# landrumb/ParlayANN

Hardware: AMD Instinct MI355X
Metric: QPS @ recall@10>=0.95, SIFT-1M d=128 beam=64; achieved HBM GB/s vs roofline (higher is better)
Workload: dtype f16; 1 GPU; SIFT-1M-shaped batched beam search: 1000000x128 integer-valued fp32->f16 base, 10000 queries/step/GPU, beam=64 k=10 cut=1.35 start=0, prebuilt Vamana R=64 L=128 alpha=1.15 x2 passes (built on device); n=1000000, d=128, nq_per_gpu=10000, beam=64, k=10, parallelism=query-sharded x1, index replicated, no collective

## Files before the change

parlayann_amd/csrc/beam_search.hip:

```cpp
#include <cstdio>
#include <cstdlib>
#include <vector>

#include "pann_device.h"

namespace pann {

#ifndef PANN_GU
#define PANN_GU 4
#endif
#ifndef PANN_GU_B128
#define PANN_GU_B128(LPC, NCH1) 4
#endif
#ifndef PANN_MINWAVES
#define PANN_MINWAVES 1
#endif
#ifndef PANN_B128_PAIR
#define PANN_B128_PAIR 0
#endif
#ifndef PANN_B128_PAIR_CODES
#define PANN_B128_PAIR_CODES 1
#endif
#ifndef PANN_B64_PREFETCH
#define PANN_B64_PREFETCH 1
// ... 375 lines not shown
          degsum += __popcll(am);
          const bool seen = filter_update<HASH_LDS>(H, hmask, act, a, lane, reinterpret_cast<uint8_t*>(Hl));
          const bool keep = act && !seen && ((int64_t)a != self);
          const uint64_t km = __ballot(keep);
          const uint32_t m = __popcll(km);
          if (keep) PANN_PL[lanes_below(km, lane)] = a;
          dcmps += m;
          PANN_WSYNC();
          PANN_STAMP(2);
          if (m) c = gather_distances<DT, METRIC, LPC, NCH1, PANN_GU>(P, qreg, qlds, PANN_PL, m, cutoff_ord, C, c, lane);
          PANN_WSYNC();
          PANN_STAMP(3);
        }
        PANN_WSYNC();
        const bool skip = (c == 0) || (P.skip_enabled && c < beam / 8 && more_unvisited);
        do_merge = !skip;
      }
      if (do_merge) {
        {
          for (uint32_t j0 = 0; j0 < c; j0 += PANN_WAVE) {
            const uint32_t j = j0 + lane;
            uint64_t key = KEY_INF;
            uint32_t p = 0;
            if (j < c) {
              key = C[j];
              bool dead = false;
              for (uint32_t i = 0; i < j; i++) dead |= (C[i] == key);
              p = lower_bound_lds(F, f, key);
              dead |= (p < f && F[p] == key);
              if (dead) key = KEY_INF;
            }
            PANN_WSYNC();
            if (j < c) { C[j] = key; CP[j] = (uint16_t)p; }
            PANN_WSYNC();
          }
          uint32_t nvalid = 0;
          for (uint32_t j0 = 0; j0 < c; j0 += PANN_WAVE) {
            const uint32_t j = j0 + lane;
            const uint64_t key = j < c ? C[j] : KEY_INF;
            nvalid += __popcll(__ballot(key != KEY_INF));
            if (key != KEY_INF) {
              uint32_t r = 0;
              for (uint32_t i = 0; i < c; i++) r += (C[i] < key) ? 1u : 0u;
              const uint32_t pos = r + CP[j];
              if (pos < beam) {
                uint32_t flag = 0u;
                for (uint32_t t = 0; t < ndrop; t++)
                  flag |= (__hip_atomic_load(DL + t, __ATOMIC_RELAXED, PANN_PRIVATE_SCOPE) == key) ? 2u : 0u;
                NF[pos] = key; NFv[pos] = (uint8_t)flag;
              }
            }
          }
          for (uint32_t e0 = 0; e0 < f; e0 += PANN_WAVE) {
            const uint32_t e = e0 + lane;
            if (e < f) {
              const uint64_t key = F[e];
              uint32_t below = 0;
              for (uint32_t i = 0; i < c; i++) below += (C[i] < key) ? 1u : 0u;
              const uint32_t pos = e + below;
              if (pos < beam) { NF[pos] = key; NFv[pos] = Fv[e]; }
            }
          }
          PANN_WSYNC();
          const uint32_t f_old = f;
          uint32_t f_new = min(f_old + nvalid, beam);
          if (!first && P.cut_enabled && f_new > P.k) {
            const float dk = key_dist(NF[P.k]);
            const float thr = (float)(P.cut * (double)dk);
            const uint64_t thr_key = (uint64_t)f2ord(thr) << 32;
            uint32_t ub = 0;
            for (uint32_t e0 = 0; e0 < f_new; e0 += PANN_WAVE) {
              const uint32_t e = e0 + lane;
              ub += __popcll(__ballot(e < f_new && NF[e] <= thr_key));
            }
            f_new = max(ub, f_old);
          }
          if (f_new == beam) {
            ndrop = 0;
          } else if (P.cut_enabled && !first) {
            for (uint32_t e0 = 0; e0 < f_old; e0 += PANN_WAVE) {
              const uint32_t e = e0 + lane;
              bool lost = false;
              uint64_t key = 0;
              if (e < f_old && Fv[e] == 1) {
                key = F[e];
                uint32_t below = 0;
                for (uint32_t i = 0; i < c; i++) below += (C[i] < key) ? 1u : 0u;
                lost = (e + below) >= f_new;
              }
              const uint64_t lm = __ballot(lost);
              if (lost) {
                const uint32_t at = ndrop + lanes_below(lm, lane);
                if (at < P.dcap) DL[at] = key; else atomicOr(P.status, 2u);
              }
              ndrop = min(ndrop + (uint32_t)__popcll(lm), P.dcap);
            }
            __builtin_amdgcn_s_waitcnt(0);
          }
          { uint64_t* t = F; F = NF; NF = t; uint8_t* tv = Fv; Fv = NFv; NFv = tv; }
          f = f_new;
          c = 0;
          PANN_WSYNC();
        }
      }
      PANN_STAMP(4);
      first = false;
    }

    const size_t qo = (size_t)qi * P.out.out_k;
    for (uint32_t j = lane; j < P.out.out_k; j += PANN_WAVE) {
      const bool ok = j < f;
      uint64_t key = 0ull;
      if (ok) key = F[j];
      if (P.out.ids) P.out.ids[qo + j] = ok ? key_id(key) : SENTINEL;
      if (P.out.dists) P.out.dists[qo + j] = ok ? key_dist(key) : __builtin_inff();
    }
#ifdef PANN_STAMPS
    if (lane == 0 && P.stamps) for (int i = 0; i < 8; i++) P.stamps[(size_t)qi * 8 + i] = stamp_sum[i];
#endif
    if (lane == 0) {
      if (P.out.frontier_size) P.out.frontier_size[qi] = f;
      if (P.out.visited_count) P.out.visited_count[qi] = nvis;
      if (P.out.dist_cmps) P.out.dist_cmps[qi] = dcmps;
      if (P.out.degree_sum) P.out.degree_sum[qi] = degsum;
    }
    PANN_WSYNC();
    if constexpr (HASH_LDS) break;
    else {
      slot = 0;
      if (lane == 0) slot = atomicAdd(P.work_counter, 1u);
      slot = __builtin_amdgcn_readfirstlane(slot);
    }
  }
}

template <int DT, int METRIC, int LPC, bool NCH1>
__global__ void __launch_bounds__(PANN_WAVE, PANN_MINWAVES_B64) beam_search_b64_kernel(BSParams P) {
  const int lane = threadIdx.x;
  extern __shared__ __align__(16) uint8_t smem[];
  uint64_t* S = reinterpret_cast<uint64_t*>(smem);
  uint64_t* C = S + 64;
  uint8_t* Sv = reinterpret_cast<uint8_t*>(C + P.ccap);
  uint4* qlds = reinterpret_cast<uint4*>(Sv + 64);
  uint32_t* H = reinterpret_cast<uint32_t*>(qlds + (NCH1 ? 0 : P.nch * LPC));
  uint32_t* Pl = reinterpret_cast<uint32_t*>(S);

  const uint32_t hsize = 1u << P.bits, hmask = hsize - 1u;
  const uint32_t beam = P.beam;
  const uint32_t BIG_ORD = f2ord(2147483648.0f);
  const uint32_t qi = P.order ? P.order[blockIdx.x] : blockIdx.x;
  if (blockIdx.x >= P.prio_start) __builtin_amdgcn_s_setprio(3);

  for (uint32_t i = lane; i < hsize; i += PANN_WAVE) H[i] = SENTINEL;
  const int64_t self = P.query_ids ? (int64_t)P.query_ids[qi] : -1;
  const uint8_t* qrow = P.query_ids ? P.points + (uint64_t)self * P.pstride : P.queries + (uint64_t)qi * P.qstride;
  QReg<DT> qreg{};
  load_query<DT, LPC, NCH1>(qrow, P.dbytes, P.nch, qreg, qlds, lane);
  PANN_WSYNC();

  uint32_t f = 0, c = 0, nvis = 0, dcmps = P.nstarts, degsum = 0, ndrop = 0;
  uint64_t fkey = KEY_INF;
  uint32_t fflag = 0;
  uint64_t* DL = P.dropped + (size_t)qi * P.dcap;
#ifdef PANN_STAMPS
  unsigned long long stamp_sum[8] = {0, 0, 0, 0, 0, 0, 0, 0}, stamp_prev;
  asm volatile("s_memtime %0\n\ts_waitcnt lgkmcnt(0)" : "=s"(stamp_prev)::"memory");
#endif

  {
    const bool act = lane < (int)P.nstarts;
    const uint32_t a = act ? P.starts[(size_t)qi * P.starts_stride + lane] : 0u;
    (void)filter_update<true>(H, hmask, act, a, lane);
    if (act) Pl[lane] = a;
    PANN_WSYNC();
    c = gather_distances<DT, METRIC, LPC, NCH1, 4>(P, qreg, qlds, Pl, P.nstarts, 0xFFFFFFFFu, C, c, lane);
    PANN_WSYNC();
  }

  uint32_t pref_id = SENTINEL, pref_row = SENTINEL;
  bool first = true;
  for (;;) {
    bool do_merge = first;
    if (!first) {
      const uint64_t um = __ballot(lane < (int)f && fflag == 0);
      if (um == 0ull || nvis >= P.limit) break;
      const int cur_idx = __ffsll((unsigned long long)um) - 1;
      const bool more_unvisited = (um & (um - 1)) != 0ull;
      PANN_STAMP(0);
      const uint64_t cur_key = readlane64(fkey, cur_idx);
      const uint32_t cur = key_id(cur_key);
      if (lane == cur_idx) fflag = 1;
      if (lane == 0 && P.out.visited_cap) {
        if (nvis < P.out.visited_cap) {
          if (P.out.visited_ids) P.out.visited_ids[(size_t)qi * P.out.visited_cap + nvis] = cur;
          if (P.out.visited_dists) P.out.visited_dists[(size_t)qi * P.out.visited_cap + nvis] = key_dist(cur_key);
        } else {
          atomicOr(P.status, 1u);
        }
      }
      nvis++;
      uint32_t cutoff_ord = BIG_ORD;
      if (f == beam) cutoff_ord = (uint32_t)(readlane64(fkey, (int)f - 1) >> 32);

      asm volatile("s_waitcnt vmcnt(0)" : "+v"(pref_row));
      const bool pref_hit = PANN_B64_PREFETCH && (pref_id == cur);
      const uint32_t pref_val = pref_row;
      pref_id = SENTINEL;
      const uint64_t rest1 = um & (um - 1);
      const bool pair_try = PANN_B64_PAIR && P.skip_enabled && rest1 != 0ull && P.gstride <= PANN_WAVE && nvis < P.limit;
      if (PANN_B64_PREFETCH) {
        const uint64_t rest = pair_try ? (rest1 & (rest1 - 1)) : rest1;
        if (rest) {
          pref_id = key_id(readlane64(fkey, __ffsll((unsigned long long)rest) - 1));
          const uint32_t* np = P.graph + (size_t)pref_id * P.gstride + min((uint32_t)lane, P.gstride - 1);
          asm volatile("global_load_dword %0, %1, off" : "=v"(pref_row) : "v"(np));
        }
      }

      const uint32_t* row = P.graph + (size_t)cur * P.gstride;
      if (pair_try) {
        const int idx2 = __ffsll((unsigned long long)rest1) - 1;
        const bool more_after2 = (rest1 & (rest1 - 1)) != 0ull;
        const uint64_t key2 = readlane64(fkey, idx2);
        const uint32_t cur2 = key_id(key2);
        uint32_t a1 = SENTINEL, a2 = SENTINEL;
        if (lane < (int)P.gstride) {
          a1 = pref_hit ? pref_val : row[lane];
          a2 = P.graph[(size_t)cur2 * P.gstride + lane];
        }
        const bool act1 = (a1 != SENTINEL) && ((uint32_t)lane < P.degree_limit);
        const bool act2 = (a2 != SENTINEL) && ((uint32_t)lane < P.degree_limit);
        PANN_STAMP(1);
        const bool seen1 = filter_update<true>(H, hmask, act1, a1, lane);
        FilterUndo u2;
        const bool seen2 = filter_update<true>(H, hmask, act2, a2, lane, nullptr, 0, LdsPart{nullptr, 0, 0}, &u2);
        const bool keep1 = act1 && !seen1 && ((int64_t)a1 != self);
        const bool keep2 = act2 && !seen2 && ((int64_t)a2 != self);
        const uint64_t km1 = __ballot(keep1), km2 = __ballot(keep2);
        const uint32_t m1 = __popcll(km1), m2 = __popcll(km2);
        const bool both = (c + m1 + m2 <= P.ccap);
        if (keep1) Pl[lanes_below(km1, lane)] = a1;
        if (both && keep2) Pl[m1 + lanes_below(km2, lane)] = a2;
        PANN_WSYNC();
        PANN_STAMP(2);
        uint32_t c_after1 = c;
        if (both) {
          if (m1 + m2) c = gather_distances_split<DT, METRIC, LPC, NCH1, PANN_GU, true>(P, qreg, qlds, Pl, m1 + m2, m1, cutoff_ord, C, c, lane, &c_after1);
        } else {
          if (m1) c = gather_distances<DT, METRIC, LPC, NCH1, PANN_GU>(P, qreg, qlds, Pl, m1, cutoff_ord, C, c, lane);
          c_after1 = c;
        }
        PANN_WSYNC();
        PANN_STAMP(3);
        const bool two = both && (c_after1 == 0 || c_after1 < beam / 8);
        if (!two) { c = c_after1; filter_undo<true>(H, u2, 0, LdsPart{nullptr, 0, 0}); }
        if (two) {
          if (lane == idx2) fflag = 1;
          if (lane == 0 && P.out.visited_cap) {
            if (nvis < P.out.visited_cap) {
              if (P.out.visited_ids) P.out.visited_ids[(size_t)qi * P.out.visited_cap + nvis] = cur2;
              if (P.out.visited_dists) P.out.visited_dists[(size_t)qi * P.out.visited_cap + nvis] = key_dist(key2);
            } else {
              atomicOr(P.status, 1u);
            }
          }
          nvis++;
        }
        degsum += __popcll(__ballot(act1)) + (two ? __popcll(__ballot(act2)) : 0u);
        dcmps += m1 + (two ? m2 : 0u);
        const bool more_left = two ? more_after2 : true;
        const bool skip = (c == 0) || (c < beam / 8 && more_left);
        do_merge = !skip;
      } else {
      for (uint32_t i0 = 0; i0 < P.gstride; i0 += PANN_WAVE) {
        const uint32_t i = i0 + lane;
        uint32_t a = SENTINEL;
        if (i0 == 0 && pref_hit) { if (i < P.gstride) a = pref_val; }
        else if (i < P.gstride) a = row[i];
        const bool act = (a != SENTINEL) && (i < P.degree_limit);
        const uint64_t am = __ballot(act);
        PANN_STAMP(1);
        if (am == 0ull) break;
        degsum += __popcll(am);
        const bool seen = filter_update<true>(H, hmask, act, a, lane);
        const bool keep = act && !seen && ((int64_t)a != self);
        const uint64_t km = __ballot(keep);
        const uint32_t m = __popcll(km);
        if (keep) Pl[lanes_below(km, lane)] = a;
        dcmps += m;
        PANN_WSYNC();
        PANN_STAMP(2);
        if (m) c = gather_distances<DT, METRIC, LPC, NCH1, PANN_GU>(P, qreg, qlds, Pl, m, cutoff_ord, C, c, lane);
        PANN_WSYNC();
        PANN_STAMP(3);
      }
      const bool skip = (c == 0) || (P.skip_enabled && c < beam / 8 && more_unvisited);
      do_merge = !skip;
      }
    }
    if (do_merge) {
      const uint32_t f_old = f;
      const bool track = P.cut_enabled && !first;
      uint32_t lt = 0;
      for (uint32_t c0 = 0; c0 < c; c0 += PANN_WAVE) {
        const uint32_t cc = min(c - c0, (uint32_t)PANN_WAVE);
        const uint64_t ckey = (lane < (int)cc) ? C[c0 + lane] : KEY_INF;
        const bool fl = lane < (int)f;
        uint32_t myp = 0, rank_c = 0, below_f = 0;
        uint64_t live_mask = 0;
        const uint64_t vmask = __ballot(fl);
        const uint32_t cid = (uint32_t)ckey, fid = (uint32_t)fkey;
        for (uint32_t i = 0; i < cc; i++) {
          const uint64_t kk = readlane64(ckey, (int)i);
          const uint32_t kid = (uint32_t)kk;
          const bool g = kk < fkey;
          const uint64_t gtm = __ballot(g);
          const uint64_t eqm = __ballot(fid == kid);
          const uint64_t dupm = __ballot(cid == kid) & ((1ull << i) - 1ull);
          if (eqm == 0ull && dupm == 0ull) {
            live_mask |= 1ull << i;
            if (lane == (int)i) myp = f - (uint32_t)__popcll(gtm & vmask);
            rank_c += (kk < ckey) ? 1u : 0u;
            below_f += g ? 1u : 0u;
          }
        }
        const uint32_t nvalid = __popcll(live_mask);
        const bool clive = (lane < (int)cc) && ((live_mask >> lane) & 1ull);
        const uint32_t cpos = rank_c + myp, fpos = (uint32_t)lane + below_f;
        if (clive && cpos < beam) {
          uint32_t flag = 0u;
          for (uint32_t t = 0; t < ndrop; t++)
            flag |= (__hip_atomic_load(DL + t, __ATOMIC_RELAXED, PANN_PRIVATE_SCOPE) == ckey) ? 2u : 0u;
          S[cpos] = ckey; Sv[cpos] = (uint8_t)flag;
        }
        if (fl && fpos < beam) { S[fpos] = fkey; Sv[fpos] = (uint8_t)fflag; }
        if (track) {
          const bool lost = fl && fflag == 1u && fpos >= beam;
          const uint64_t lm = __ballot(lost);
          if (lost) {
            const uint32_t at = ndrop + lt + lanes_below(lm, lane);
            if (at < P.dcap) DL[at] = fkey; else atomicOr(P.status, 2u);
          }
          lt += __popcll(lm);
        }
        PANN_WSYNC();
        f = min(f + nvalid, beam);
        fkey = (lane < (int)f) ? S[lane] : KEY_INF;
        fflag = (lane < (int)f) ? (uint32_t)Sv[lane] : 0u;
        PANN_WSYNC();
      }
      uint32_t f_new = f;
      if (!first && P.cut_enabled && f_new > P.k) {
        const float dk = key_dist(readlane64(fkey, (int)P.k));
        const float thr = (float)(P.cut * (double)dk);
        const uint64_t thr_key = (uint64_t)f2ord(thr) << 32;
        const uint32_t ub = __popcll(__ballot(lane < (int)f_new && fkey <= thr_key));
        f_new = max(ub, f_old);
      }
      if (f_new == beam) {
        ndrop = 0;
      } else if (track) {
        const bool lost = lane >= (int)f_new && lane < (int)f && fflag == 1u;
        const uint64_t lm = __ballot(lost);
        if (lost) {
          const uint32_t at = ndrop + lt + lanes_below(lm, lane);
          if (at < P.dcap) DL[at] = fkey; else atomicOr(P.status, 2u);
        }
        lt += __popcll(lm);
        ndrop = min(ndrop + lt, P.dcap);
        if (lt) __builtin_amdgcn_s_waitcnt(0);
      }
      f = f_new;
      if (lane >= (int)f) { fkey = KEY_INF; fflag = 0u; }
      c = 0;
    }
    PANN_STAMP(4);
    first = false;
  }
  asm volatile("s_waitcnt vmcnt(0)" : "+v"(pref_row));

  const size_t qo = (size_t)qi * P.out.out_k;
  if (lane < (int)P.out.out_k) {
    const bool ok = lane < (int)f;
    if (P.out.ids) P.out.ids[qo + lane] = ok ? key_id(fkey) : SENTINEL;
    if (P.out.dists) P.out.dists[qo + lane] = ok ? key_dist(fkey) : __builtin_inff();
  }
#ifdef PANN_STAMPS
  if (lane == 0 && P.stamps) for (int i = 0; i < 8; i++) P.stamps[(size_t)qi * 8 + i] = stamp_sum[i];
#endif
  if (lane == 0) {
    if (P.out.frontier_size) P.out.frontier_size[qi] = f;
    if (P.out.visited_count) P.out.visited_count[qi] = nvis;
    if (P.out.dist_cmps) P.out.dist_cmps[qi] = dcmps;
    if (P.out.degree_sum) P.out.degree_sum[qi] = degsum;
  }
}

template <int DT, int METRIC, int LPC, bool NCH1, bool HASH_LDS, bool CODES = false>
__global__ void __launch_bounds__(PANN_WAVE) beam_search_b128_kernel(BSParams P) {
  static_assert(!CODES || HASH_LDS, "the code table lives in LDS");
  constexpr int RB = 2;
  const int lane = threadIdx.x;
  extern __shared__ __align__(16) uint8_t smem[];
  uint64_t* S = reinterpret_cast<uint64_t*>(smem);
  uint64_t* C = S + 64 * RB;
  uint8_t* Sv = reinterpret_cast<uint8_t*>(C + P.ccap);
  uint4* qlds = reinterpret_cast<uint4*>(Sv + 64 * RB);
  uint32_t* Hl = reinterpret_cast<uint32_t*>(qlds + (NCH1 ? 0 : P.nch * LPC));
  uint8_t* T = reinterpret_cast<uint8_t*>(S);
  uint32_t* Pl = reinterpret_cast<uint32_t*>(S);

  const uint32_t hsize = 1u << P.bits, hmask = hsize - 1u;
  const uint32_t beam = P.beam;
  const uint32_t BIG_ORD = f2ord(2147483648.0f);
  const LdsPart Lp{reinterpret_cast<uint8_t*>(Hl), HASH_LDS ? 0u : (P.hsplit == 3 ? hsize : P.hsplit ? hsize - (hsize >> P.hsplit) : 0u), P.p24};
  uint32_t slot = blockIdx.x;
  if constexpr (!HASH_LDS) {
    slot = 0;
    if (lane == 0) slot = atomicAdd(P.work_counter, 1u);
    slot = __builtin_amdgcn_readfirstlane(slot);
  }
  while (slot < P.nq) {
  const uint32_t qi = P.order ? P.order[slot] : slot;
  uint32_t* H = HASH_LDS ? Hl : P.hash_global + ((size_t)blockIdx.x << P.bits);
  const uint32_t hb = HASH_LDS ? 0u : P.hsplit;
  uint8_t* const P8 = reinterpret_cast<uint8_t*>(Hl);
  uint32_t* const P4 = Hl + (hsize >> 2);
  if constexpr (CODES) {
    for (uint32_t i = lane; i < (hsize >> 2) + (hsize >> 3); i += PANN_WAVE) Hl[i] = 0xFFFFFFFFu;
  } else {
    if (hb != 3) for (uint32_t i = lane; i < (hsize >> hb); i += PANN_WAVE) hstore<HASH_LDS>(H, i, SENTINEL);
    if (hb) lds_part_clear(Lp, lane);
  }
  const int64_t self = P.query_ids ? (int64_t)P.query_ids[qi] : -1;
  const uint8_t* qrow = P.query_ids ? P.points + (uint64_t)self * P.pstride : P.queries + (uint64_t)qi * P.qstride;
  QReg<DT> qreg{};
  load_query<DT, LPC, NCH1>(qrow, P.dbytes, P.nch, qreg, qlds, lane);
  hsync<HASH_LDS>();

  uint32_t f = 0, c = 0, nvis = 0, dcmps = P.nstarts, degsum = 0, ndrop = 0;
  uint64_t fkey[RB] = {KEY_INF, KEY_INF};
  uint32_t fflag[RB] = {0, 0};
  uint64_t* DL = P.dropped + (size_t)qi * P.dcap;
#ifdef PANN_STAMPS
  unsigned long long stamp_sum[8] = {0, 0, 0, 0, 0, 0, 0, 0}, stamp_prev;
  asm volatile("s_memtime %0\n\ts_waitcnt lgkmcnt(0)" : "=s"(stamp_prev)::"memory");
#endif
  auto entry_key = [&](uint32_t e) -> uint64_t {
    return (e < 64) ? readlane64(fkey[0], (int)e) : readlane64(fkey[1], (int)e - 64);
  };

  {
    const bool act = lane < (int)P.nstarts;
    const uint32_t a = act ? P.starts[(size_t)qi * P.starts_stride + lane] : 0u;
    if constexpr (CODES) (void)filter_update_codes(P8, P4, hmask, act, a, act ? (uint32_t)P.rank16[a] : 0u, lane, T);
    else (void)filter_update<HASH_LDS>(H, hmask, act, a, lane, T, hb, Lp);
    if (act) Pl[lane] = a;
    PANN_WSYNC();
    c = gather_distances<DT, METRIC, LPC, NCH1, 4, false>(P, qreg, qlds, Pl, P.nstarts, 0xFFFFFFFFu, C, c, lane);
    PANN_WSYNC();
  }

  uint32_t pref_id = SENTINEL, pref_row = SENTINEL, pref_code = 0;
  bool first = true;
  for (;;) {
    bool do_merge = first;
    if (!first) {
      const uint64_t um0 = __ballot(lane < (int)f && fflag[0] == 0);
      const uint64_t um1 = __ballot(lane + 64 < (int)f && fflag[1] == 0);
      if ((um0 | um1) == 0ull || nvis >= P.limit) break;
      const int cur_idx = um0 ? __ffsll((unsigned long long)um0) - 1 : 64 + __ffsll((unsigned long long)um1) - 1;
      const bool more_unvisited = (__popcll(um0) + __popcll(um1)) > 1;
      PANN_STAMP(0);
      const uint64_t cur_key = entry_key((uint32_t)cur_idx);
      const uint32_t cur = key_id(cur_key);
      if ((CODES ? PANN_B128_PAIR_CODES : PANN_B128_PAIR) && P.skip_enabled && more_unvisited && P.gstride <= PANN_WAVE && nvis + 1 < P.limit) {
        uint64_t r0 = um0, r1 = um1;
        if (r0) r0 &= r0 - 1; else r1 &= r1 - 1;
        const int idx2 = r0 ? __ffsll((unsigned long long)r0) - 1 : 64 + __ffsll((unsigned long long)r1) - 1;
        if (r0) r0 &= r0 - 1; else r1 &= r1 - 1;
        const bool more_after2 = (r0 | r1) != 0ull;
        const uint64_t key2 = entry_key((uint32_t)idx2);
        const uint32_t cur2 = key_id(key2);
        uint32_t cutoff2 = BIG_ORD;
        if (f == beam) cutoff2 = (uint32_t)(entry_key(f - 1) >> 32);
        uint32_t a1 = SENTINEL, a2 = SENTINEL, code1 = 0, code2 = 0;
        if (lane < (int)P.gstride) {
          a1 = (pref_id == cur) ? pref_row : P.graph[(size_t)cur * P.gstride + lane];
          a2 = P.graph[(size_t)cur2 * P.gstride + lane];
          if constexpr (CODES) {
            code1 = (pref_id == cur) ? pref_code : (uint32_t)P.gcode[(size_t)cur * P.gstride + lane];
            code2 = P.gcode[(size_t)cur2 * P.gstride + lane];
          }
        }
        pref_id = SENTINEL;
        const bool act1 = (a1 != SENTINEL) && ((uint32_t)lane < P.degree_limit);
        const bool act2 = (a2 != SENTINEL) && ((uint32_t)lane < P.degree_limit);
        FilterUndo u2;
        bool seen1, seen2;
        if constexpr (CODES) {
          seen1 = filter_update_codes(P8, P4, hmask, act1, a1, code1, lane, T);
          seen2 = filter_update_codes(P8, P4, hmask, act2, a2, code2, lane, T, &u2);
        } else {
          seen1 = filter_update<HASH_LDS>(H, hmask, act1, a1, lane, T, hb, Lp);
          seen2 = filter_update<HASH_LDS>(H, hmask, act2, a2, lane, T, hb, Lp, &u2);
        }
        const bool keep1 = act1 && !seen1 && ((int64_t)a1 != self);
        const bool keep2 = act2 && !seen2 && ((int64_t)a2 != self);
        const uint64_t km1 = __ballot(keep1), km2 = __ballot(keep2);
        const uint32_t m1 = __popcll(km1), m2 = __popcll(km2);
        const bool both = (c + m1 + m2 <= P.ccap);
        if (keep1) Pl[lanes_below(km1, lane)] = a1;
        if (both && keep2) Pl[m1 + lanes_below(km2, lane)] = a2;
        PANN_WSYNC();
        uint32_t c_after1 = c;
        if (both) {
          if (m1 + m2) c = gather_distances_split<DT, METRIC, LPC, NCH1, PANN_GU_B128(LPC, NCH1)>(P, qreg, qlds, Pl, m1 + m2, m1, cutoff2, C, c, lane, &c_after1);
        } else {
          if (m1) c = gather_distances<DT, METRIC, LPC, NCH1, PANN_GU_B128(LPC, NCH1), false>(P, qreg, qlds, Pl, m1, cutoff2, C, c, lane);
          c_after1 = c;
        }
        PANN_WSYNC();
        const bool two = both && (c_after1 == 0 || c_after1 < beam / 8);
        if (!two) {
          c = c_after1;
          if constexpr (CODES) filter_undo_codes(P8, P4, u2);
          else filter_undo<HASH_LDS>(H, u2, hb, Lp);
        }
        if (cur_idx < 64) { if (lane == cur_idx) fflag[0] = 1; } else { if (lane == cur_idx - 64) fflag[1] = 1; }
        if (two) { if (idx2 < 64) { if (lane == idx2) fflag[0] = 1; } else { if (lane == idx2 - 64) fflag[1] = 1; } }
        if (lane == 0 && P.out.visited_cap) {
          const uint32_t nv = two ? 2u : 1u;
          if (nvis + nv <= P.out.visited_cap) {
            const size_t at = (size_t)qi * P.out.visited_cap + nvis;
            if (P.out.visited_ids) { P.out.visited_ids[at] = cur; if (two) P.out.visited_ids[at + 1] = cur2; }
            if (P.out.visited_dists) { P.out.visited_dists[at] = key_dist(cur_key); if (two) P.out.visited_dists[at + 1] = key_dist(key2); }
          } else {
            atomicOr(P.status, 1u);
          }
        }
        nvis += two ? 2u : 1u;
        degsum += __popcll(__ballot(act1)) + (two ? __popcll(__ballot(act2)) : 0u);
        dcmps += m1 + (two ? m2 : 0u);
        const bool more_left = two ? more_after2 : true;
        const bool skip = (c == 0) || (c < beam / 8 && more_left);
        do_merge = !skip;
      } else {
      if (cur_idx < 64) { if (lane == cur_idx) fflag[0] = 1; } else { if (lane == cur_idx - 64) fflag[1] = 1; }
      if (lane == 0 && P.out.visited_cap) {
        if (nvis < P.out.visited_cap) {
          if (P.out.visited_ids) P.out.visited_ids[(size_t)qi * P.out.visited_cap + nvis] = cur;
          if (P.out.visited_dists) P.out.visited_dists[(size_t)qi * P.out.visited_cap + nvis] = key_dist(cur_key);
        } else {
          atomicOr(P.status, 1u);
        }
      }
      nvis++;
      uint32_t cutoff_ord = BIG_ORD;
      if (f == beam) cutoff_ord = (uint32_t)(entry_key(f - 1) >> 32);

      const uint32_t* row = P.graph + (size_t)cur * P.gstride;
      const uint16_t* crow = CODES ? P.gcode + (size_t)cur * P.gstride : nullptr;
      const bool pref_hit = (pref_id == cur);
      const uint32_t pref_val = pref_row, pref_cval = pref_code;
      uint32_t next_id = SENTINEL;
      {
        uint64_t r0 = um0, r1 = um1;
        if (r0) r0 &= r0 - 1; else r1 &= r1 - 1;
        if (r0 | r1) {
          const int nx = r0 ? __ffsll((unsigned long long)r0) - 1 : 64 + __ffsll((unsigned long long)r1) - 1;
          next_id = key_id(entry_key((uint32_t)nx));
        }
      }
      pref_id = SENTINEL;
      for (uint32_t i0 = 0; i0 < P.gstride; i0 += PANN_WAVE) {
        const uint32_t i = i0 + lane;
        uint32_t a = SENTINEL, code = 0;
        if (i0 == 0 && pref_hit) { a = pref_val; code = pref_cval; }
        else if (i < P.gstride) { a = row[i]; if constexpr (CODES) code = crow[i]; }
        const bool act = (a != SENTINEL) && (i < P.degree_limit);
        const uint64_t am = __ballot(act);
        PANN_STAMP(1);
        if (am == 0ull) break;
        degsum += __popcll(am);
        bool seen;
        if constexpr (CODES) seen = filter_update_codes(P8, P4, hmask, act, a, code, lane, T);
        else seen = filter_update<HASH_LDS>(H, hmask, act, a, lane, T, hb, Lp);
        const bool keep = act && !seen && ((int64_t)a != self);
        const uint64_t km = __ballot(keep);
        const uint32_t m = __popcll(km);
        if (keep) Pl[lanes_below(km, lane)] = a;
        dcmps += m;
        PANN_WSYNC();
        PANN_STAMP(2);
        if (i0 == 0 && next_id != SENTINEL && P.query_ids) {
          pref_id = next_id;
          pref_row = (lane < (int)P.gstride) ? P.graph[(size_t)next_id * P.gstride + lane] : SENTINEL;
          if constexpr (CODES) pref_code = (lane < (int)P.gstride) ? (uint32_t)P.gcode[(size_t)next_id * P.gstride + lane] : 0u;
        }
        if (m) c = gather_distances<DT, METRIC, LPC, NCH1, PANN_GU_B128(LPC, NCH1), false>(P, qreg, qlds, Pl, m, cutoff_ord, C, c, lane);
        PANN_WSYNC();
        PANN_STAMP(3);
      }
      const bool skip = (c == 0) || (P.skip_enabled && c < beam / 8 && more_unvisited);
      do_merge = !skip;
      }
    }
    if (do_merge) {
      const uint32_t f_old = f;
      const bool track = P.cut_enabled && !first;
      uint32_t lt = 0;
      for (uint32_t c0 = 0; c0 < c; c0 += PANN_WAVE) {
        const uint32_t cc = min(c - c0, (uint32_t)PANN_WAVE);
        const uint64_t ckey = (lane < (int)cc) ? C[c0 + lane] : KEY_INF;
        const bool fl[RB] = {lane < (int)f, lane + 64 < (int)f};
        uint32_t myp = 0, rank_c = 0, below_f[RB] = {0, 0};
        uint64_t live_mask = 0;
        const uint64_t vmask0 = __ballot(fl[0]), vmask1 = __ballot(fl[1]);
        const uint32_t cid = (uint32_t)ckey, fid0 = (uint32_t)fkey[0], fid1 = (uint32_t)fkey[1];
        for (uint32_t i = 0; i < cc; i++) {
          const uint64_t kk = readlane64(ckey, (int)i);
          const uint32_t kid = (uint32_t)kk;
          const bool g0 = kk < fkey[0], g1 = kk < fkey[1];
          const uint64_t gt0 = __ballot(g0), gt1 = __ballot(g1);
          const uint64_t eqm = __ballot(fid0 == kid || fid1 == kid);
          const uint64_t dupm = __ballot(cid == kid) & ((1ull << i) - 1ull);
          if (eqm == 0ull && dupm == 0ull) {
            live_mask |= 1ull << i;
            if (lane == (int)i) myp = f - (uint32_t)__popcll(gt0 & vmask0) - (uint32_t)__popcll(gt1 & vmask1);
            rank_c += (kk < ckey) ? 1u : 0u;
            below_f[0] += g0 ? 1u : 0u;
            below_f[1] += g1 ? 1u : 0u;
          }
        }
        const uint32_t nvalid = __popcll(live_mask);
        const bool clive = (lane < (int)cc) && ((live_mask >> lane) & 1ull);
        const uint32_t cpos = rank_c + myp;
        if (clive && cpos < beam) {
          uint32_t flag = 0u;
          for (uint32_t t = 0; t < ndrop; t++)
            flag |= (__hip_atomic_load(DL + t, __ATOMIC_RELAXED, PANN_PRIVATE_SCOPE) == ckey) ? 2u : 0u;
          S[cpos] = ckey; Sv[cpos] = (uint8_t)flag;
        }
#pragma unroll
        for (int r = 0; r < RB; r++) {
          const uint32_t fpos = (uint32_t)lane + 64 * r + below_f[r];
          if (fl[r] && fpos < beam) { S[fpos] = fkey[r]; Sv[fpos] = (uint8_t)fflag[r]; }
          if (track) {
            const bool lost = fl[r] && fflag[r] == 1u && fpos >= beam;
            const uint64_t lm = __ballot(lost);
            if (lost) {
              const uint32_t at = ndrop + lt + lanes_below(lm, lane);
              if (at < P.dcap) DL[at] = fkey[r]; else atomicOr(P.status, 2u);
            }
            lt += __popcll(lm);
          }
        }
        PANN_WSYNC();
        f = min(f + nvalid, beam);
#pragma unroll
        for (int r = 0; r < RB; r++) {
          const bool in = lane + 64 * r < (int)f;
          fkey[r] = in ? S[lane + 64 * r] : KEY_INF;
          fflag[r] = in ? (uint32_t)Sv[lane + 64 * r] : 0u;
        }
        PANN_WSYNC();
      }
      uint32_t f_new = f;
      if (!first && P.cut_enabled && f_new > P.k) {
        const float dk = key_dist(entry_key(P.k));
        const float thr = (float)(P.cut * (double)dk);
        const uint64_t thr_key = (uint64_t)f2ord(thr) << 32;
        const uint32_t ub = __popcll(__ballot(lane < (int)f_new && fkey[0] <= thr_key)) +
                            __popcll(__ballot(lane + 64 < (int)f_new && fkey[1] <= thr_key));
        f_new = max(ub, f_old);
      }
      if (f_new == beam) {
        ndrop = 0;
      } else if (track) {
#pragma unroll
        for (int r = 0; r < RB; r++) {
          const int e = lane + 64 * r;
          const bool lost = e >= (int)f_new && e < (int)f && fflag[r] == 1u;
          const uint64_t lm = __ballot(lost);
          if (lost) {
            const uint32_t at = ndrop + lt + lanes_below(lm, lane);
            if (at < P.dcap) DL[at] = fkey[r]; else atomicOr(P.status, 2u);
          }
          lt += __popcll(lm);
        }
        ndrop = min(ndrop + lt, P.dcap);
        if (lt) __builtin_amdgcn_s_waitcnt(0);
      }
      f = f_new;
#pragma unroll
      for (int r = 0; r < RB; r++) if (lane + 64 * r >= (int)f) { fkey[r] = KEY_INF; fflag[r] = 0u; }
      c = 0;
    }
    PANN_STAMP(4);
    first = false;
  }
#ifdef PANN_STAMPS
  if (lane == 0 && P.stamps) for (int i = 0; i < 8; i++) P.stamps[(size_t)qi * 8 + i] = stamp_sum[i];
#endif

  const size_t qo = (size_t)qi * P.out.out_k;
#pragma unroll
  for (int r = 0; r < RB; r++) {
    const uint32_t j = lane + 64 * r;
    if (j < P.out.out_k) {
      const bool ok = j < f;
      if (P.out.ids) P.out.ids[qo + j] = ok ? key_id(fkey[r]) : SENTINEL;
      if (P.out.dists) P.out.dists[qo + j] = ok ? key_dist(fkey[r]) : __builtin_inff();
    }
  }
  if (lane == 0) {
    if (P.out.frontier_size) P.out.frontier_size[qi] = f;
    if (P.out.visited_count) P.out.visited_count[qi] = nvis;
    if (P.out.dist_cmps) P.out.dist_cmps[qi] = dcmps;
    if (P.out.degree_sum) P.out.degree_sum[qi] = degsum;
  }
  if constexpr (HASH_LDS) {
    break;
  } else {
    PANN_WSYNC();
    if (lane == 0) slot = atomicAdd(P.work_counter, 1u);
    slot = __builtin_amdgcn_readfirstlane(slot);
  }
  }
}


void choose_point_layout(uint32_t dbytes, uint32_t* lpc, uint32_t* nch) {
  const uint32_t r64 = (dbytes + 63) / 64 * 64;
  if (const char* f = ab_env("PANN_FORCE_LPC")) {
    const uint32_t l = (uint32_t)atoi(f);
    if ((l == 4 || l == 8 || l == 16) && r64 % (l * 16) == 0 && r64 / (l * 16) > 1) { *lpc = l; *nch = r64 / (l * 16); return; }
  }
  if (r64 == 128) { *lpc = 8; *nch = 1; return; }
  if (r64 == 256) { *lpc = 16; *nch = 1; return; }
  if (r64 == 512) { *lpc = 32; *nch = 1; return; }
  if (r64 % 256 == 0) { *lpc = 16; *nch = r64 / 256; return; }
  if (r64 % 128 == 0) { *lpc = 8; *nch = r64 / 128; return; }
  *lpc = 4; *nch = r64 / 64;
}

static uint32_t filter_bits(int64_t beam) {
  double l = std::ceil(std::log2((double)beam * (double)beam)) - 2.0;
  int b = (int)l;
  return (uint32_t)(b < 10 ? 10 : b);
}

struct Plan {
  uint32_t bits, bcap, ccap, deg_eff, dcap, lds_bytes; bool hash_lds; uint32_t slots; bool b64; bool b128;
  bool b128_codes;
  bool b128_hbm;
  uint32_t hsplit;
  uint32_t p24;
};

static Plan make_plan(const DeviceIndex& ix, const SearchArgs& a) {
  Plan p;
  p.bits = filter_bits(a.beam);
  const uint32_t beam = (uint32_t)a.beam;
  p.bcap = (std::max<uint32_t>(beam, a.nstarts) + 63) / 64 * 64;
  int64_t dl = std::min<int64_t>(std::max<int64_t>(a.degree_limit, 0), (int64_t)ix.max_deg);
  p.deg_eff = (uint32_t)dl;
  p.ccap = (std::max<uint32_t>(beam / 8 + p.deg_eff, a.nstarts) + 63) / 64 * 64;
  p.dcap = std::max<uint32_t>(a.dcap, 64);
  const bool nch1 = layout_query_in_registers(ix);
  size_t fixed = (size_t)p.bcap * 8 * 2 + (size_t)p.ccap * 8 + (size_t)p.bcap * 2 +
                 (size_t)p.ccap * 2 + (nch1 ? 0 : (size_t)ix.nch * ix.lpc * 16);
  size_t hbytes = (size_t)4 << p.bits;
  p.hash_lds = (hbytes <= 16384) && (fixed + hbytes <= 64 * 1024);
  p.lds_bytes = (uint32_t)(fixed + (p.hash_lds ? hbytes : 1024));
  p.slots = 256 * 8;
  p.b64 = p.hash_lds && p.bcap == 64;
  if (p.b64) {
    p.ccap = (std::max<uint32_t>(beam / 8 + p.deg_eff, a.nstarts) + 7) / 8 * 8;
    p.lds_bytes = (uint32_t)(64 * 8 + (size_t)p.ccap * 8 + 64 + (nch1 ? 0 : (size_t)ix.nch * ix.lpc * 16) + hbytes);
  }
  p.b128 = p.hash_lds && p.bcap == 128 && a.nstarts <= 64;
  p.b128_hbm = false;
  p.b128_codes = p.b128 && p.bits == FILTER_CODE_BITS && ix.codes_valid && ix.gcode && ix.rank16 && ix.gstride <= PANN_WAVE;
  if (p.b128_codes) {
    p.ccap = (std::max<uint32_t>(beam / 8 + p.deg_eff, a.nstarts) + 7) / 8 * 8;
    p.hsplit = 0; p.p24 = 0;
    p.lds_bytes = (uint32_t)(128 * 8 + (size_t)p.ccap * 8 + 128 + (nch1 ? 0 : (size_t)ix.nch * ix.lpc * 16) + ((size_t)1 << p.bits) * 3 / 2);
  } else if (p.b128) {
    p.ccap = (std::max<uint32_t>(beam / 8 + p.deg_eff, a.nstarts) + 7) / 8 * 8;
    static const bool force_lds = ab_env("PANN_B128_LDS") != nullptr;
    p.b128_hbm = (hbytes > 8192) && a.nq > 2048 && !force_lds;
    p.hsplit = 0;
    if (p.b128_hbm) {
      static const char* sp = ab_env("PANN_B128_SPLIT");
      p.hsplit = sp ? (uint32_t)atoi(sp) : 1u;
      if (p.hsplit > 3) p.hsplit = 0;
      static const bool no24 = ab_env("PANN_B128_NO24") != nullptr;
      if (p.hsplit == 3 && (no24 || !(ix.n < 0xFFFFFFull))) p.hsplit = 1;
      p.hash_lds = false; p.slots = 256 * 32;
      p.p24 = (p.hsplit && ix.n < 0xFFFFFFull && !no24) ? 1u : 0u;
      hbytes = p.hsplit == 3 ? ((size_t)3 << p.bits)
             : p.hsplit ? (((size_t)1 << p.bits) - ((size_t)1 << (p.bits - p.hsplit))) * (p.p24 ? 3 : 4) : 0;
    }
    p.lds_bytes = (uint32_t)(128 * 8 + (size_t)p.ccap * 8 + 128 + (nch1 ? 0 : (size_t)ix.nch * ix.lpc * 16) + hbytes);
  }
  return p;
}

size_t search_workspace_bytes(const DeviceIndex& ix, const SearchArgs& a) {
  Plan p = make_plan(ix, a);
  size_t need = 256;
  need += (size_t)a.nq * p.dcap * 8;
  if (!p.hash_lds) need += ((size_t)std::min<uint64_t>(a.nq, p.slots) << p.bits) * 4;
  return need;
}

template <int DT, int METRIC, int LPC, bool NCH1>
static hipError_t launch_variant(const BSParams& P, const Plan& p, hipStream_t stream) {
  if (p.b64) {
    auto kern = beam_search_b64_kernel<DT, METRIC, LPC, NCH1>;
    hipLaunchKernelGGL(kern, dim3(P.nq), dim3(PANN_WAVE), p.lds_bytes, stream, P);
  } else if (p.b128_codes) {
    auto kern = beam_search_b128_kernel<DT, METRIC, LPC, NCH1, true, true>;
    hipLaunchKernelGGL(kern, dim3(P.nq), dim3(PANN_WAVE), p.lds_bytes, stream, P);
  } else if (p.b128) {
    if (p.b128_hbm) {
      auto kern = beam_search_b128_kernel<DT, METRIC, LPC, NCH1, false>;
      const uint32_t grid = (uint32_t)std::min<uint64_t>(P.nq, p.slots);
      hipLaunchKernelGGL(kern, dim3(grid), dim3(PANN_WAVE), p.lds_bytes, stream, P);
    } else {
      auto kern = beam_search_b128_kernel<DT, METRIC, LPC, NCH1, true>;
      hipLaunchKernelGGL(kern, dim3(P.nq), dim3(PANN_WAVE), p.lds_bytes, stream, P);
    }
  } else if (p.hash_lds) {
    auto kern = beam_search_kernel<DT, METRIC, LPC, NCH1, true>;
    if (p.lds_bytes > 48 * 1024)
      (void)hipFuncSetAttribute(reinterpret_cast<const void*>(kern), hipFuncAttributeMaxDynamicSharedMemorySize, (int)p.lds_bytes);
    hipLaunchKernelGGL(kern, dim3(P.nq), dim3(PANN_WAVE), p.lds_bytes, stream, P);
  } else {
    auto kern = beam_search_kernel<DT, METRIC, LPC, NCH1, false>;
    if (p.lds_bytes > 48 * 1024)
      (void)hipFuncSetAttribute(reinterpret_cast<const void*>(kern), hipFuncAttributeMaxDynamicSharedMemorySize, (int)p.lds_bytes);
    const uint32_t grid = (uint32_t)std::min<uint64_t>(P.nq, p.slots);
    hipLaunchKernelGGL(kern, dim3(grid), dim3(PANN_WAVE), p.lds_bytes, stream, P);
  }
  return hipGetLastError();
}

template <int DT, int METRIC>
static hipError_t launch_layout(const DeviceIndex& ix, const BSParams& P, const Plan& p, hipStream_t s) {
  if (layout_query_in_registers(ix)) {
    if (ix.lpc == 8) return launch_variant<DT, METRIC, 8, true>(P, p, s);
    if (ix.lpc == 16) return launch_variant<DT, METRIC, 16, true>(P, p, s);
    if (ix.lpc == 32) return launch_variant<DT, METRIC, 32, true>(P, p, s);
  }
  if (ix.lpc == 4) return launch_variant<DT, METRIC, 4, false>(P, p, s);
  if (ix.lpc == 8) return launch_variant<DT, METRIC, 8, false>(P, p, s);
  if (ix.lpc == 16) return launch_variant<DT, METRIC, 16, false>(P, p, s);
  return hipErrorInvalidValue;
}

int launch_beam_search(const DeviceIndex& ix, const SearchArgs& a, void* ws, size_t ws_bytes,
                       hipStream_t stream) {
  if (a.nq == 0) return PANN_OK;
  if (a.nq > 0xFFFFFFF0ull) { set_error("pann_batch_search: nq too large"); return PANN_ERR_BAD_ARG; }
  if (a.beam <= 0 || a.beam > 65536) { set_error("pann_batch_search: beam out of range [1,65536]"); return PANN_ERR_BAD_ARG; }
  if (a.nstarts == 0) {
    set_error("beam search expects at least one start point"); return PANN_ERR_BAD_ARG;
  }
  if ((int64_t)a.nstarts > a.beam) { set_error("pann_batch_search: more start points than beam"); return PANN_ERR_BAD_ARG; }
  if (a.out.out_k > (uint64_t)a.beam) {
    set_error("Error: beam search parameter Q same size or smaller than k"); return PANN_ERR_BAD_ARG;
  }
  if ((a.queries == nullptr) == (a.query_ids == nullptr)) {
    set_error("pann_batch_search: exactly one of queries / query_ids must be given"); return PANN_ERR_BAD_ARG;
  }
  Plan p = make_plan(ix, a);
  if (p.lds_bytes > 160 * 1024) { set_error("pann_batch_search: beam/degree too large for LDS state"); return PANN_ERR_UNSUPPORTED; }
  if (search_workspace_bytes(ix, a) > ws_bytes) { set_error("pann_batch_search: workspace too small"); return PANN_ERR_BAD_ARG; }

  BSParams P;
  P.points = ix.points; P.pstride = ix.pstride; P.dbytes = ix.dbytes; P.nch = ix.nch; P.exact = ix.exact;
  P.graph = ix.graph; P.gstride = ix.gstride; P.max_deg = ix.max_deg;
  P.queries = a.queries; P.qstride = a.qstride; P.query_ids = a.query_ids;
  P.starts = a.starts; P.nstarts = a.nstarts; P.starts_stride = a.starts_per_query ? a.nstarts : 0u; P.nq = (uint32_t)a.nq;
  P.k = (uint32_t)std::max<int64_t>(a.k, 0); P.beam = (uint32_t)a.beam;
  P.limit = (uint32_t)std::min<int64_t>(std::max<int64_t>(a.limit, 0), 0xFFFFFFFFll);
  P.degree_limit = p.deg_eff; P.cut = a.cut;
  P.skip_enabled = (a.limit >= 2 * a.beam) ? 1u : 0u;
  P.cut_enabled = (a.k > 0 && ix.metric == PANN_L2) ? 1u : 0u;
  P.bits = p.bits; P.bcap = p.bcap; P.ccap = p.ccap;
  uint8_t* w = (uint8_t*)ws;
  P.work_counter = (uint32_t*)w; P.status = (uint32_t*)(w + 64);
  P.dropped = (uint64_t*)(w + 256); P.dcap = p.dcap;
  {
    static const char* pf = ab_env("PANN_PRIO_FROM");
    const uint32_t tenths = pf ? (uint32_t)atoi(pf) : 8u;
    P.prio_start = tenths >= 10 ? 0xFFFFFFFFu : (uint32_t)((uint64_t)a.nq * tenths / 10);
  }
  P.hsplit = p.b128_hbm ? p.hsplit : 0u;
  P.p24 = p.b128_hbm ? p.p24 : 0u;
  P.gcode = ix.gcode; P.rank16 = ix.rank16;
  P.order = a.order;
  P.hash_global = p.hash_lds ? nullptr : (uint32_t*)(w + 256 + (size_t)a.nq * p.dcap * 8);
  P.out = a.out;
  P.stamps = nullptr;
#ifdef PANN_STAMPS
  static unsigned long long* d_stamps = nullptr; static size_t stamps_cap = 0;
  if (stamps_cap < a.nq) { if (d_stamps) (void)hipFree(d_stamps); (void)hipMalloc((void**)&d_stamps, a.nq * 64); stamps_cap = a.nq; }
  P.stamps = d_stamps;
#endif
  PANN_HIP(hipMemsetAsync(w, 0, 256, stream));

  hipError_t e = hipErrorInvalidValue;
#define PANN_DISPATCH(DT, MT) if (ix.dtype == DT && ix.metric == MT) e = launch_layout<DT, MT>(ix, P, p, stream);
  PANN_DISPATCH(PANN_U8, PANN_L2) PANN_DISPATCH(PANN_U8, PANN_MIPS)
  PANN_DISPATCH(PANN_I8, PANN_L2) PANN_DISPATCH(PANN_I8, PANN_MIPS)
  PANN_DISPATCH(PANN_F32, PANN_L2) PANN_DISPATCH(PANN_F32, PANN_MIPS)
  PANN_DISPATCH(PANN_F16, PANN_L2) PANN_DISPATCH(PANN_F16, PANN_MIPS)
  PANN_DISPATCH(PANN_BF16, PANN_L2) PANN_DISPATCH(PANN_BF16, PANN_MIPS)
#undef PANN_DISPATCH
  if (e != hipSuccess) return hip_fail(e, "beam_search_kernel launch");
  if (a.out.status) PANN_HIP(hipMemcpyAsync(a.out.status, P.status, 4, hipMemcpyDeviceToDevice, stream));
#ifdef PANN_STAMPS
  if (ab_env("PANN_STAMPS_PRINT") && a.nq >= 1000) {
    (void)hipStreamSynchronize(stream);
    std::vector<unsigned long long> h(a.nq * 8);
    (void)hipMemcpy(h.data(), P.stamps, a.nq * 64, hipMemcpyDeviceToHost);
    double sum[8] = {0}; for (size_t q = 0; q < a.nq; q++) for (int i = 0; i < 8; i++) sum[i] += (double)h[q * 8 + i];
    double tot = 0; for (int i = 0; i < 5; i++) tot += sum[i];
    fprintf(stderr, "[stamps] per-query cycles: head %.0f row %.0f filter %.0f gather %.0f merge %.0f total %.0f  (shares %.1f%% %.1f%% %.1f%% %.1f%% %.1f%%)\n",
            sum[0] / a.nq, sum[1] / a.nq, sum[2] / a.nq, sum[3] / a.nq, sum[4] / a.nq, tot / a.nq, 100 * sum[0] / tot, 100 * sum[1] / tot,
            100 * sum[2] / tot, 100 * sum[3] / tot, 100 * sum[4] / tot);
  }
#endif
  return PANN_OK;
}

}
```

Baseline: 7.398 million queries/s.

## Rewrite beam merge with LDS-scan ranking and fast path, keep ballot fallback

Replaces the per-candidate ballot loop in the frontier/candidate merge with a per-lane scan over candidate keys read from LDS in pairs. Each lane computes its rank and the frontier's shift directly, and duplicates against the frontier are corrected afterwards. It then writes the merged beam through LDS using a flag bit, and falls back to the original ballot-based merge only when the fast merge leaves gaps, for example from duplicates within the candidate chunk. The goal is to remove the cross-lane ballots and readlanes per candidate in the merge phase. The cost is extra LDS traffic, more synchronisation and code complexity. It also adds stamp counters for merge statistics.

```diff
diff --git a/parlayann_amd/csrc/beam_search.hip b/parlayann_amd/csrc/beam_search.hip
--- a/parlayann_amd/csrc/beam_search.hip
+++ b/parlayann_amd/csrc/beam_search.hip
@@ -701,51 +701,112 @@
       const uint32_t f_old = f;
       const bool track = P.cut_enabled && !first;
       uint32_t lt = 0;
-      for (uint32_t c0 = 0; c0 < c; c0 += PANN_WAVE) {
-        const uint32_t cc = min(c - c0, (uint32_t)PANN_WAVE);
-        const uint64_t ckey = (lane < (int)cc) ? C[c0 + lane] : KEY_INF;
-        const bool fl = lane < (int)f;
-        uint32_t myp = 0, rank_c = 0, below_f = 0;
-        uint64_t live_mask = 0;
-        const uint64_t vmask = __ballot(fl);
-        const uint32_t cid = (uint32_t)ckey, fid = (uint32_t)fkey;
-        for (uint32_t i = 0; i < cc; i++) {
-          const uint64_t kk = readlane64(ckey, (int)i);
-          const uint32_t kid = (uint32_t)kk;
-          const bool g = kk < fkey;
-          const uint64_t gtm = __ballot(g);
-          const uint64_t eqm = __ballot(fid == kid);
-          const uint64_t dupm = __ballot(cid == kid) & ((1ull << i) - 1ull);
-          if (eqm == 0ull && dupm == 0ull) {
-            live_mask |= 1ull << i;
-            if (lane == (int)i) myp = f - (uint32_t)__popcll(gtm & vmask);
-            rank_c += (kk < ckey) ? 1u : 0u;
-            below_f += g ? 1u : 0u;
-          }
-        }
-        const uint32_t nvalid = __popcll(live_mask);
-        const bool clive = (lane < (int)cc) && ((live_mask >> lane) & 1ull);
-        const uint32_t cpos = rank_c + myp, fpos = (uint32_t)lane + below_f;
-        if (clive && cpos < beam) {
-          uint32_t flag = 0u;
-          for (uint32_t t = 0; t < ndrop; t++)
-            flag |= (__hip_atomic_load(DL + t, __ATOMIC_RELAXED, PANN_PRIVATE_SCOPE) == ckey) ? 2u : 0u;
-          S[cpos] = ckey; Sv[cpos] = (uint8_t)flag;
-        }
-        if (fl && fpos < beam) { S[fpos] = fkey; Sv[fpos] = (uint8_t)fflag; }
-        if (track) {
+      const uint32_t cu = __builtin_amdgcn_readfirstlane(c);
+      for (uint32_t c0 = 0; c0 < cu; c0 += PANN_WAVE) {
+        const uint32_t cc = min(cu - c0, (uint32_t)PANN_WAVE);
+        const uint32_t cc2 = (cc + 1u) & ~1u;
+        const uint32_t fu = __builtin_amdgcn_readfirstlane(f);
+        uint64_t* Cc = C + c0;
+        int ml = lane;
+        asm volatile("" : "+v"(ml));
+        const uint64_t ckey = (ml < (int)cc) ? Cc[ml] : KEY_INF;
+        const bool fl = ml < (int)fu;
+        const uint32_t fid = (uint32_t)fkey;
+        Sv[ml] = 0;
+        if (ml >= (int)cc && ml < (int)cc2) Cc[ml] = KEY_INF;
+        PANN_WSYNC();
+        uint32_t rank_c = 0, below_f = 0;
+        bool hit = false;
+        for (uint32_t i = 0; i < cc; i += 2) {
+          const uint4 kp = *reinterpret_cast<const uint4*>(Cc + i);
+          const uint64_t k0 = ((uint64_t)kp.y << 32) | kp.x, k1 = ((uint64_t)kp.w << 32) | kp.z;
+          below_f += (k0 < fkey ? 1u : 0u) + (k1 < fkey ? 1u : 0u);
+          rank_c += (k0 < ckey ? 1u : 0u) + (k1 < ckey ? 1u : 0u);
+          hit |= (kp.x == fid) | (kp.z == fid);
+        }
+        const uint64_t hm = __ballot(fl && hit);
+        bool cdead = false;
+        for (uint64_t m = hm; m; m &= m - 1ull) {
+          const uint64_t x = readlane64(fkey, __ffsll((unsigned long long)m) - 1);
+          rank_c -= (x < ckey) ? 1u : 0u;
+          below_f -= (x < fkey) ? 1u : 0u;
+          cdead |= (ckey == x);
+        }
+        const uint32_t nf = min(fu + cc - (uint32_t)__popcll(hm), beam);
+        const uint32_t fpos_fast = (uint32_t)ml + below_f;
+        PANN_WSYNC();
+        if (ml < (int)cc2) Cc[ml] = KEY_INF;
+        if (ml < (int)cc && !cdead) Cc[rank_c] = ckey;
+        if (fl && fpos_fast < beam) { S[fpos_fast] = fkey; Sv[fpos_fast] = (uint8_t)(fflag | 4u); }
+        PANN_WSYNC();
+        const bool in = ml < (int)nf;
+        const bool from_f = (Sv[ml] & 4u) != 0u;
+        const uint64_t occ = __ballot(from_f);
+        const uint64_t nkey = !in ? KEY_INF : from_f ? S[ml] : Cc[min(lanes_below(~occ, ml), cc - 1u)];
+        const bool fast = __ballot(in && nkey == KEY_INF) == 0ull;
+#ifdef PANN_STAMPS
+        stamp_sum[5] += cc;
+        stamp_sum[6] += fast ? 0u : 1u;
+        stamp_sum[7] += (uint32_t)__popcll(hm);
+#endif
+        auto track_lost = [&](uint32_t fpos) {
+          if (!track) return;
           const bool lost = fl && fflag == 1u && fpos >= beam;
           const uint64_t lm = __ballot(lost);
           if (lost) {
-            const uint32_t at = ndrop + lt + lanes_below(lm, lane);
+            const uint32_t at = ndrop + lt + lanes_below(lm, ml);
             if (at < P.dcap) DL[at] = fkey; else atomicOr(P.status, 2u);
           }
           lt += __popcll(lm);
-        }
-        PANN_WSYNC();
-        f = min(f + nvalid, beam);
-        fkey = (lane < (int)f) ? S[lane] : KEY_INF;
-        fflag = (lane < (int)f) ? (uint32_t)Sv[lane] : 0u;
+        };
+        if (fast) {
+          track_lost(fpos_fast);
+          uint32_t flag = Sv[ml] & 3u;
+          if (in && !from_f) {
+            flag = 0u;
+            for (uint32_t t = 0; t < ndrop; t++)
+              flag |= (__hip_atomic_load(DL + t, __ATOMIC_RELAXED, PANN_PRIVATE_SCOPE) == nkey) ? 2u : 0u;
+          }
+          f = nf;
+          fkey = nkey;
+          fflag = in ? flag : 0u;
+        } else {
+          const uint64_t ckey = (ml < (int)cc) ? Cc[ml] : KEY_INF;
+          uint32_t myp = 0;
+          uint64_t live_mask = 0;
+          rank_c = 0; below_f = 0;
+          const uint64_t vmask = __ballot(fl);
+          const uint32_t cid = (uint32_t)ckey;
+          for (uint32_t i = 0; i < cc; i++) {
+            const uint64_t kk = readlane64(ckey, (int)i);
+            const uint32_t kid = (uint32_t)kk;
+            const bool g = kk < fkey;
+            const uint64_t gtm = __ballot(g);
+            const uint64_t eqm = __ballot(fid == kid);
+            const uint64_t dupm = __ballot(cid == kid) & ((1ull << i) - 1ull);
+            if (eqm == 0ull && dupm == 0ull && kk != KEY_INF) {
+              live_mask |= 1ull << i;
+              if (ml == (int)i) myp = fu - (uint32_t)__popcll(gtm & vmask);
+              rank_c += (kk < ckey) ? 1u : 0u;
+              below_f += g ? 1u : 0u;
+            }
+          }
+          const uint32_t nvalid = __popcll(live_mask);
+          const bool clive = (ml < (int)cc) && ((live_mask >> ml) & 1ull);
+          const uint32_t cpos = rank_c + myp, fpos = (uint32_t)ml + below_f;
+          if (clive && cpos < beam) {
+            uint32_t flag = 0u;
+            for (uint32_t t = 0; t < ndrop; t++)
+              flag |= (__hip_atomic_load(DL + t, __ATOMIC_RELAXED, PANN_PRIVATE_SCOPE) == ckey) ? 2u : 0u;
+            S[cpos] = ckey; Sv[cpos] = (uint8_t)flag;
+          }
+          if (fl && fpos < beam) { S[fpos] = fkey; Sv[fpos] = (uint8_t)fflag; }
+          track_lost(fpos);
+          PANN_WSYNC();
+          f = min(fu + nvalid, beam);
+          fkey = (ml < (int)f) ? S[ml] : KEY_INF;
+          fflag = (ml < (int)f) ? (uint32_t)Sv[ml] : 0u;
+        }
         PANN_WSYNC();
       }
       uint32_t f_new = f;
@@ -1332,6 +1393,12 @@
     fprintf(stderr, "[stamps] per-query cycles: head %.0f row %.0f filter %.0f gather %.0f merge %.0f total %.0f  (shares %.1f%% %.1f%% %.1f%% %.1f%% %.1f%%)\n",
             sum[0] / a.nq, sum[1] / a.nq, sum[2] / a.nq, sum[3] / a.nq, sum[4] / a.nq, tot / a.nq, 100 * sum[0] / tot, 100 * sum[1] / tot,
             100 * sum[2] / tot, 100 * sum[3] / tot, 100 * sum[4] / tot);
+    if (p.b64) {
+      unsigned long long mx = 0; for (size_t q = 0; q < a.nq; q++) mx = h[q * 8 + 5] > mx ? h[q * 8 + 5] : mx;
+      fprintf(stderr, "[stamps] merged candidates per query: mean %.1f max %llu; merge cycles per candidate %.1f; "
+              "slow-path chunks per query %.4f; in-frontier candidates per query %.2f\n",
+              sum[5] / a.nq, mx, sum[5] ? sum[4] / sum[5] : 0.0, sum[6] / a.nq, sum[7] / a.nq);
+    }
   }
 #endif
   return PANN_OK;
```

Measured after the change: 7.464 million queries/s (median of 5 runs). No clear change (+0.9%).
